# JeffWang987/MVSTER

Measured on AMD Instinct MI355X. Metric: depth-maps/sec (DTU 512×640, 5-view, 4-stage) at 1/2/4/8 MI355X, higher is better.
Workload: dtype f32; 1 GPU; DTU mid 512x640, 5 views, 4-stage cascade 8/8/4/4 hyp, B=1 eval, 1 depth map(s) per step per GPU; launch=hipGraph replay, parallelism=replicas x1, depth_maps_in_flight_per_gpu=2

## Files before the change

mvster_amd/csrc/conv_pers.hip:

```cpp
#include "conv_args.hpp"

namespace mvconv {
namespace {


#ifdef MVSTER_TIMELINE
__device__ unsigned long long* g_ptl = nullptr;
#define MV_PTL(k)                                                                                                       \
    do {                                                                                                                \
        __builtin_amdgcn_sched_barrier(0);                                                                              \
        if (g_ptl && lane == 0 && it < 16)                                                                              \
            g_ptl[(((size_t)(blockIdx.y * gridDim.x + blockIdx.x) * 4 + wave) * 16 + it) * 8 + (k)] =                    \
                (k) < 5 ? __builtin_amdgcn_s_memtime() : (k) == 5 ? __builtin_amdgcn_s_getreg(63492)                    \
                                                         : (k) == 6 ? __builtin_amdgcn_s_getreg(63508) : tile;          \
        __builtin_amdgcn_sched_barrier(0);                                                                              \
    } while (0)
#define MV_PPTL(k, v)                                                                                                   \
    do {                                                                                                                \
        __builtin_amdgcn_sched_barrier(0);                                                                              \
        if (g_ptl && lane == 0 && hp < 16)                                                                              \
            g_ptl[(((size_t)(blockIdx.y * gridDim.x + blockIdx.x) * 8 + wave8) * 16 + hp) * 4 + (k)] = (v);           \
        __builtin_amdgcn_sched_barrier(0);                                                                              \
    } while (0)
#else
// ... 571 lines not shown
                    const int tap = dy * kw + dx;
#pragma unroll
                    for (int c = 0; c < NCH; ++c) {
                        const f32x4v w = wl[(wbase + tap * NCH + c) * 64 + lane];
                        f32x4v A[MT];
#pragma unroll
                        for (int mt = 0; mt < MT; ++mt) A[mt] = patch[abase[mt] + c * 2 * PLANE + cbase + dy * RS + dx * 2];
#pragma unroll
                        for (int j = 0; j < 4; ++j)
#pragma unroll
                            for (int mt = 0; mt < MT; ++mt) acc[mt] = __builtin_amdgcn_mfma_f32_16x16x4f32(w[j], A[mt][j], acc[mt], 0, 0, 0);
                    }
                }
            wbase += kh * kw * NCH;
#pragma unroll
            for (int mt = 0; mt < MT; ++mt) {
                f32x4v v = acc[mt];
#pragma unroll
                for (int j = 0; j < 4; ++j) {
                    v[j] = fmaf(v[j], scv[j], shv[j]);
                    if (a.relu) v[j] = fmaxf(v[j], 0.0f);
                    if (SKIP) v[j] += skv[mt][j];
                }
                __builtin_amdgcn_raw_buffer_store_b128(__builtin_bit_cast(u32x4v, v), out_rsrc, ooff[mt], 0, MV_STORE_AUX);
            }
        }
        __builtin_amdgcn_s_waitcnt(0xc07f);
        __builtin_amdgcn_s_barrier();
    }
}

#ifdef MVSTER_PROBES
template <int MT, int NT, int KW, int SW, int NCH, int KD, bool WREG, int PF, bool SKIP>
__global__ void __launch_bounds__(512) conv_pp_kernel(ConvArgs a, PersArgs p) {
    using G = PersGeom<MT, KW, SW, KD>;
    constexpr int TY = G::TY, KH = G::KH, PW = G::PW, PH = G::PH, PWH = G::PWH, PLANE = G::PLANE, NBLK = G::NBLK;
    constexpr int NTAP = KD * KH * KW, TAPS2D = KH * KW;
    constexpr int BUF = NCH * 2 * PLANE;
    constexpr int NI = NCH * 2 * NBLK;
    constexpr int NIW = (NI + 3) / 4;
    constexpr int CIN = NCH * 16;
    extern __shared__ __attribute__((aligned(16))) float lds_raw[];
    const int lane = threadIdx.x & 63;
    const int wave8 = __builtin_amdgcn_readfirstlane(threadIdx.x >> 6);
    const int grp = wave8 >> 2;
    const int wave = wave8 & 3;
    f32x4v* const lds = reinterpret_cast<f32x4v*>(lds_raw) + grp * 2 * BUF;
    f32x4v* const scratch = reinterpret_cast<f32x4v*>(lds_raw) + 4 * BUF;
    f32x4v* const wl = scratch + 64;
    const int lm = lane & 15, lq = lane >> 4;
    const int nt0 = blockIdx.y * NT;
    const __amdgpu_buffer_rsrc_t in_rsrc =
        __builtin_amdgcn_make_buffer_rsrc(const_cast<float*>(a.in), (short)0, (int)a.in_bytes, 0x00020000);

    unsigned dbase[NIW];
    int dpos[NIW];
#pragma unroll
    for (int n = 0; n < NIW; ++n) {
        const int i = wave + 4 * n;
        const int c = i / (2 * NBLK), r = i - c * 2 * NBLK, pl = r / NBLK, blk = r - pl * NBLK;
        const int s = blk * 64 + lane;
        const int q1 = s & 1;
        int prow, px;
        if (SW == 1) {
            const int pix = s >> 1;
            prow = pix / PW;
            px = pix - prow * PW;
        } else {
            int t = s >> 1;
            const int xh = t % PWH;
            t /= PWH;
            prow = t >> 1;
            px = 2 * xh + (t & 1);
        }
        const bool valid = i < NI && prow < G::ROWS && px < PW;
        const int pz = KD == 1 ? 0 : prow / PH, py = prow - pz * PH;
        dpos[n] = px | (py << 8) | (pz << 16);
        dbase[n] = valid ? (unsigned)(((pz * a.Hi + py) * a.Wi + px) * (CIN * 4) + (c * 16 + pl * 8 + q1 * 4) * 4) : 0x80000000u;
    }

    auto decode_tile = [&](unsigned tile) -> TilePos {
        TilePos t;
        auto div = [&](unsigned n, int k) -> unsigned { return ((__umulhi(n, p.mul[k]) >> p.shr[k]) & ~p.one[k]) | (n & p.one[k]); };
        unsigned q = div(tile, 0);
        t.tx0 = (int)(tile - q * p.tiles_x) * 32;
        unsigned q2 = div(q, 1);
        t.ty0 = (int)(q - q2 * p.tiles_y) * TY;
        const unsigned q3 = div(q2, 2);
        t.zo = (int)(q2 - q3 * (unsigned)a.Do);
        t.b = (int)q3;
        return t;
    };

    auto dma_tile = [&](const TilePos& t, int buf, bool live) {
        const int iz0 = t.zo * a.sd - a.pd[0], iy0 = t.ty0 * SW - a.ph[0], ix0 = t.tx0 * SW - a.pw[0];
        const unsigned origin = (unsigned)((((t.b * a.Di + iz0) * a.Hi + iy0) * a.Wi + ix0) * (CIN * 4));
        const unsigned wi = live ? (unsigned)a.Wi : 0u;
        f32x4v* const dst0 = lds + buf * BUF;
#pragma unroll
        for (int n = 0; n < NIW; ++n) {
            const int i = wave + 4 * n;
            {
                const int ix = ix0 + (dpos[n] & 255), iy = iy0 + ((dpos[n] >> 8) & 255), iz = iz0 + (dpos[n] >> 16);
                bool ok = (unsigned)iy < (unsigned)a.Hi && (unsigned)ix < wi;
                if (KD > 1) ok = ok && (unsigned)iz < (unsigned)a.Di;
                const unsigned off = ok ? dbase[n] + origin : 0x80000000u;
                f32x4v* const dst = (NI % 4 == 0 || n + 1 < NIW || i < NI) ? dst0 + (i / NBLK) * PLANE + (i % NBLK) * 64 : scratch;
                __builtin_amdgcn_raw_ptr_buffer_load_lds(in_rsrc, (lds_void*)dst, 16, off, 0, 0, 0);
            }
        }
    };

    const unsigned nwg = gridDim.x;
    const unsigned first = xcd_remap(blockIdx.x, nwg);
    const unsigned ntl = first < p.ntiles ? (p.ntiles - first + nwg - 1) / nwg : 0u;
    const int kcount = (int)((ntl + 1u - (unsigned)grp) >> 1);
    auto tile_of = [&](int k) -> unsigned { return first + (unsigned)(2 * k + grp) * nwg; };
    if (kcount > 0) dma_tile(decode_tile(tile_of(0)), 0, true);
    if (grp == 0 && kcount > 1) dma_tile(decode_tile(tile_of(1)), 1, true);
    f32x4v wreg[WREG ? NTAP * NCH * NT : 1];
    const long wstep = (long)a.ntile_total * 256;
    if (WREG) {
#pragma unroll
        for (int s = 0; s < NTAP * NCH; ++s)
#pragma unroll
            for (int nt = 0; nt < NT; ++nt)
                wreg[s * NT + nt] = *reinterpret_cast<const f32x4v*>(a.wpk + s * wstep + ((long)(nt0 + nt) * 64 + lane) * 4);
    } else {
        const __amdgpu_buffer_rsrc_t w_rsrc = __builtin_amdgcn_make_buffer_rsrc(
            const_cast<float*>(a.wpk), (short)0, (int)(NTAP * NCH * wstep * 4), 0x00020000);
        for (int i = wave8; i < NTAP * NCH * NT; i += 8) {
            const int s = i / NT, nt = i - s * NT;
            const unsigned off = (unsigned)((s * wstep + (long)(nt0 + nt) * 256) * 4) + lane * 16;
            __builtin_amdgcn_raw_ptr_buffer_load_lds(w_rsrc, (lds_void*)(wl + i * 64), 16, off, 0, 0, 0);
        }
    }
    f32x4v scv[NT], shv[NT];
#pragma unroll
    for (int nt = 0; nt < NT; ++nt) {
        const int n0 = (nt0 + nt) * 16 + lq * 4;
        scv[nt] = *reinterpret_cast<const f32x4v*>(a.scale + n0);
        shv[nt] = *reinterpret_cast<const f32x4v*>(a.shift + n0);
    }
    int abase[MT];
#pragma unroll
    for (int mt = 0; mt < MT; ++mt) {
        const int t = wave * MT + mt;
        const int row = t >> 1, x = (t & 1) * 16 + lm;
        const int rs = G::ROWSLOTS;
        abase[mt] = (SW == 1 ? row * rs + x * 2 : row * 2 * rs + x * 2) + (lq >> 1) * PLANE + (lq & 1);
    }
    const __amdgpu_buffer_rsrc_t out_rsrc =
        __builtin_amdgcn_make_buffer_rsrc(a.out, (short)0, (int)p.out_bytes, 0x00020000);
    const __amdgpu_buffer_rsrc_t skip_rsrc = __builtin_amdgcn_make_buffer_rsrc(
        const_cast<float*>(SKIP ? a.skip : a.in), (short)0, SKIP ? (int)p.out_bytes : 0, 0x00020000);
    unsigned obase[MT];
    int orc[MT];
#pragma unroll
    for (int mt = 0; mt < MT; ++mt) {
        const int t = wave * MT + mt;
        const int row = t >> 1, col = (t & 1) * 16 + lm;
        orc[mt] = row | (col << 8);
        obase[mt] = (unsigned)((row * a.Wo + col) * a.cout + nt0 * 16 + lq * 4) * 4u;
    }
    auto tap_off = [&](int kz, int ky, int kx) -> int {
        const int prow = kz * PH + ky;
        return SW == 1 ? prow * G::ROWSLOTS + kx * 2 : prow * G::ROWSLOTS + (kx & 1) * PWH * 2 + (kx >> 1) * 2;
    };

    __syncthreads();

    f32x4v pacc[MT][NT], pskv[MT][NT];
    unsigned pooff[MT];
#pragma unroll
    for (int mt = 0; mt < MT; ++mt) {
        pooff[mt] = 0x80000000u;
#pragma unroll
        for (int nt = 0; nt < NT; ++nt) pacc[mt][nt] = pskv[mt][nt] = (f32x4v){0.f, 0.f, 0.f, 0.f};
    }
    auto epilogue = [&](const f32x4v (&accv)[MT][NT], const f32x4v (&skvv)[MT][NT], const unsigned (&off)[MT]) {
#pragma unroll
        for (int mt = 0; mt < MT; ++mt) {
#pragma unroll
            for (int nt = 0; nt < NT; ++nt) {
                f32x4v v = accv[mt][nt];
#pragma unroll
                for (int j = 0; j < 4; ++j) {
                    v[j] = fmaf(v[j], scv[nt][j], shv[nt][j]);
                    if (a.relu) v[j] = fmaxf(v[j], 0.0f);
                    if (SKIP) v[j] += skvv[mt][nt][j];
                }
                __builtin_amdgcn_raw_buffer_store_b128(__builtin_bit_cast(u32x4v, v), out_rsrc, off[mt] + nt * 64, 0, MV_STORE_AUX);
            }
        }
    };

    f32x4v skvN[MT][NT];
    unsigned ooffN[MT];
    TilePos here = decode_tile(kcount > 0 ? tile_of(0) : 0u);
#pragma unroll
    for (int mt = 0; mt < MT; ++mt) ooffN[mt] = 0x80000000u;
    const int nhalf = 2 * (int)((ntl + 1u) >> 1) + 1;
    {
        const unsigned oorigin = (unsigned)((((here.b * a.Do + here.zo) * a.Ho + here.ty0) * a.Wo + here.tx0) * a.cout) * 4u;
#pragma unroll
        for (int mt = 0; mt < MT; ++mt) {
            const bool ok = grp == 0 && kcount > 0 && here.ty0 + (orc[mt] & 255) < a.Ho && here.tx0 + (orc[mt] >> 8) < a.Wo;
            ooffN[mt] = ok ? obase[mt] + oorigin : 0x80000000u;
#pragma unroll
            for (int nt = 0; nt < NT; ++nt)
                skvN[mt][nt] = SKIP ? __builtin_bit_cast(f32x4v, __builtin_amdgcn_raw_buffer_load_b128(skip_rsrc, ooffN[mt] + nt * 64, 0, 0))
                                    : (f32x4v){0.f, 0.f, 0.f, 0.f};
        }
    }
    for (int hp = 0; hp < nhalf; ++hp) {
        MV_PPTL(0, __builtin_amdgcn_s_memtime());
        MV_PPTL(3, __builtin_amdgcn_s_getreg(63492));
        if ((hp & 1) == grp) {
            const int k = (hp - grp) >> 1;
            if (k < kcount) {
                const int cur = k & 1;
                f32x4v acc[MT][NT];
#pragma unroll
                for (int mt = 0; mt < MT; ++mt)
#pragma unroll
                    for (int nt = 0; nt < NT; ++nt) acc[mt][nt] = (f32x4v){0.f, 0.f, 0.f, 0.f};
                const f32x4v* patch = lds + cur * BUF;
                const int kz_lo = KD == 1 ? 0 : max(0, a.pd[0] - here.zo * a.sd), kz_hi = KD == 1 ? 1 : min(KD, a.Di + a.pd[0] - here.zo * a.sd);
#pragma unroll
                for (int kz = 0; kz < KD; ++kz) {
                    if (kz < kz_lo || kz >= kz_hi) continue;
                    f32x4v A[PF + 1][NCH][MT], Bv[PF + 1][NCH][NT];
                    auto load_tap = [&](int t2, f32x4v (&Aa)[NCH][MT], f32x4v (&Bb)[NCH][NT]) {
                        const int ky = t2 / KW, kx = t2 - ky * KW;
                        const int to = tap_off(kz, ky, kx);
                        const int tap = kz * TAPS2D + t2;
#pragma unroll
                        for (int c = 0; c < NCH; ++c) {
#pragma unroll
                            for (int mt = 0; mt < MT; ++mt) Aa[c][mt] = patch[abase[mt] + c * 2 * PLANE + to];
#pragma unroll
                            for (int nt = 0; nt < NT; ++nt)
                                Bb[c][nt] = WREG ? wreg[(tap * NCH + c) * NT + nt] : wl[((tap * NCH + c) * NT + nt) * 64 + lane];
                        }
                    };
#pragma unroll
                    for (int t2 = 0; t2 < PF && t2 < TAPS2D; ++t2) load_tap(t2, A[t2 % (PF + 1)], Bv[t2 % (PF + 1)]);
#pragma unroll
                    for (int t2 = 0; t2 < TAPS2D; ++t2) {
                        if (t2 + PF < TAPS2D) load_tap(t2 + PF, A[(t2 + PF) % (PF + 1)], Bv[(t2 + PF) % (PF + 1)]);
#pragma unroll
                        for (int c = 0; c < NCH; ++c)
#pragma unroll
                            for (int j = 0; j < 4; ++j)
#pragma unroll
                                for (int mt = 0; mt < MT; ++mt)
#pragma unroll
                                    for (int nt = 0; nt < NT; ++nt)
                                        acc[mt][nt] = __builtin_amdgcn_mfma_f32_16x16x4f32(Bv[t2 % (PF + 1)][c][nt][j], A[t2 % (PF + 1)][c][mt][j],
                                                                                           acc[mt][nt], 0, 0, 0);
                    }
                }
#pragma unroll
                for (int mt = 0; mt < MT; ++mt) {
                    pooff[mt] = ooffN[mt];
#pragma unroll
                    for (int nt = 0; nt < NT; ++nt) {
                        pacc[mt][nt] = acc[mt][nt];
                        pskv[mt][nt] = skvN[mt][nt];
                    }
                }
            }
            __builtin_amdgcn_s_waitcnt(0xc07f);
            MV_PPTL(2, k < kcount ? 1 : 0);
        } else {
            const int kn = (hp + 1 - grp) >> 1;
            epilogue(pacc, pskv, pooff);
#pragma unroll
            for (int mt = 0; mt < MT; ++mt) pooff[mt] = 0x80000000u;
            __builtin_amdgcn_sched_barrier(0);
            const bool have = kn < kcount;
            here = decode_tile(have ? tile_of(kn) : 0u);
            const unsigned oorigin = (unsigned)((((here.b * a.Do + here.zo) * a.Ho + here.ty0) * a.Wo + here.tx0) * a.cout) * 4u;
#pragma unroll
            for (int mt = 0; mt < MT; ++mt) {
                const bool ok = have && here.ty0 + (orc[mt] & 255) < a.Ho && here.tx0 + (orc[mt] >> 8) < a.Wo;
                ooffN[mt] = ok ? obase[mt] + oorigin : 0x80000000u;
#pragma unroll
                for (int nt = 0; nt < NT; ++nt)
                    skvN[mt][nt] = SKIP ? __builtin_bit_cast(f32x4v, __builtin_amdgcn_raw_buffer_load_b128(skip_rsrc, ooffN[mt] + nt * 64, 0, 0))
                                        : (f32x4v){0.f, 0.f, 0.f, 0.f};
            }
            __builtin_amdgcn_sched_barrier(0);
            const bool more = kn + 1 < kcount;
            dma_tile(decode_tile(more ? tile_of(kn + 1) : 0u), (kn + 1) & 1, more);
            MV_PPTL(2, __builtin_amdgcn_s_memtime());
            asm volatile("s_waitcnt vmcnt(%0)" ::"n"(MT * NT * (SKIP ? 2 : 1) + NIW) : "memory");
        }
        MV_PPTL(1, __builtin_amdgcn_s_memtime());
        __builtin_amdgcn_s_barrier();
    }
}
#endif

template <int NCH, int MT>
__global__ void __launch_bounds__(256) conv1x1_pers_kernel(ConvArgs a, unsigned ngroups, unsigned mtot, unsigned out_bytes) {
    constexpr int CIN = NCH * 16;
    extern __shared__ __attribute__((aligned(16))) float lds_raw[];
    f32x4v* const wl = reinterpret_cast<f32x4v*>(lds_raw);
    const int ntile = a.ntile_total;
    f32x4v* const ssl = wl + NCH * ntile * 64;
    const int lane = threadIdx.x & 63;
    const int wave = __builtin_amdgcn_readfirstlane(threadIdx.x >> 6);
    const int lm = lane & 15, lq = lane >> 4;
    const __amdgpu_buffer_rsrc_t in_rsrc =
        __builtin_amdgcn_make_buffer_rsrc(const_cast<float*>(a.in), (short)0, (int)a.in_bytes, 0x00020000);
    const __amdgpu_buffer_rsrc_t out_rsrc = __builtin_amdgcn_make_buffer_rsrc(a.out, (short)0, (int)out_bytes, 0x00020000);
    const __amdgpu_buffer_rsrc_t skip_rsrc = __builtin_amdgcn_make_buffer_rsrc(
        const_cast<float*>(a.skip_mode ? a.skip : a.in), (short)0,
        a.skip_mode == 1 ? (int)out_bytes : a.skip_mode == 2 ? (int)(out_bytes / 4) : 0, 0x00020000);
    {
        const __amdgpu_buffer_rsrc_t w_rsrc =
            __builtin_amdgcn_make_buffer_rsrc(const_cast<float*>(a.wpk), (short)0, NCH * ntile * 1024, 0x00020000);
        for (int i = wave; i < NCH * ntile; i += 4) {
            const unsigned off = (unsigned)(i * 1024 + lane * 16);
            f32x4v* const dst = wl + i * 64;
            __builtin_amdgcn_raw_ptr_buffer_load_lds(w_rsrc, (lds_void*)dst, 16, off, 0, 0, 0);
        }
        for (int i = threadIdx.x; i < ntile * 4; i += 256) {
            ssl[i] = *reinterpret_cast<const f32x4v*>(a.scale + i * 4);
            ssl[ntile * 4 + i] = *reinterpret_cast<const f32x4v*>(a.shift + i * 4);
        }
    }
    auto load_group = [&](unsigned g, f32x4v (&A)[MT][NCH], unsigned (&vox)[MT]) {
#pragma unroll
        for (int mt = 0; mt < MT; ++mt) {
            const unsigned m = ((g * 4 + wave) * MT + mt) * 16 + lm;
            vox[mt] = m;
#pragma unroll
            for (int c = 0; c < NCH; ++c) {
                const unsigned off = m < mtot ? (m * CIN + c * 16 + lq * 4) * 4u : 0x80000000u;
                A[mt][c] = __builtin_bit_cast(f32x4v, __builtin_amdgcn_raw_buffer_load_b128(in_rsrc, off, 0, 0));
            }
        }
    };
    f32x4v A[MT][NCH], An[MT][NCH];
    unsigned vox[MT], voxn[MT];
    struct Up {
        unsigned o00, o01, o10, o11;
        mv::Lerp ly, lx;
    } up[MT];
    unsigned g = blockIdx.x;
    if (g < ngroups) load_group(g, A, vox);
    __syncthreads();
    const unsigned cout4 = (unsigned)a.cout * 4u;
    for (; g < ngroups; g += gridDim.x) {
        const unsigned gn = g + gridDim.x < ngroups ? g + gridDim.x : g;
        load_group(gn, An, voxn);
        if (a.skip_mode == 2) {
            const int hh = a.HoF / 2, wh = a.WoF / 2;
#pragma unroll
            for (int mt = 0; mt < MT; ++mt) {
                const unsigned m = vox[mt] < mtot ? vox[mt] : 0u;
                const unsigned t = fast_div(m, (unsigned)a.Wo, a.div_mul[0], a.div_shr[0]);
                const int ox = (int)(m - t * (unsigned)a.Wo);
                const unsigned b = fast_div(t, (unsigned)a.Ho, a.div_mul[1], a.div_shr[1]);
                const int oy = (int)(t - b * (unsigned)a.Ho);
                up[mt].ly = mv::make_lerp(oy, hh, a.HoF);
                up[mt].lx = mv::make_lerp(ox, wh, a.WoF);
                const unsigned base = b * (unsigned)(hh * wh);
                up[mt].o00 = (base + up[mt].ly.i0 * wh + up[mt].lx.i0) * cout4;
                up[mt].o01 = (base + up[mt].ly.i0 * wh + up[mt].lx.i1) * cout4;
                up[mt].o10 = (base + up[mt].ly.i1 * wh + up[mt].lx.i0) * cout4;
                up[mt].o11 = (base + up[mt].ly.i1 * wh + up[mt].lx.i1) * cout4;
            }
        }
        f32x4v Bv[NCH];
#pragma unroll
        for (int c = 0; c < NCH; ++c) Bv[c] = wl[(c * ntile) * 64 + lane];
        for (int nt = 0; nt < ntile; ++nt) {
            f32x4v Bn[NCH];
            const int ntn = nt + 1 < ntile ? nt + 1 : nt;
#pragma unroll
            for (int c = 0; c < NCH; ++c) Bn[c] = wl[(c * ntile + ntn) * 64 + lane];
            const f32x4v sc = ssl[nt * 4 + lq], sh = ssl[ntile * 4 + nt * 4 + lq];
            f32x4v acc[MT];
#pragma unroll
            for (int mt = 0; mt < MT; ++mt) acc[mt] = (f32x4v){0.f, 0.f, 0.f, 0.f};
#pragma unroll
            for (int c = 0; c < NCH; ++c)
#pragma unroll
                for (int j = 0; j < 4; ++j)
#pragma unroll
                    for (int mt = 0; mt < MT; ++mt)
                        acc[mt] = __builtin_amdgcn_mfma_f32_16x16x4f32(Bv[c][j], A[mt][c][j], acc[mt], 0, 0, 0);
            const unsigned n0 = (unsigned)(nt * 16 + lq * 4);
#pragma unroll
            for (int mt = 0; mt < MT; ++mt) {
                const unsigned off = (n0 < (unsigned)a.cout && vox[mt] < mtot) ? vox[mt] * cout4 + n0 * 4u : 0x80000000u;
                f32x4v v = acc[mt];
#pragma unroll
                for (int j = 0; j < 4; ++j) {
                    v[j] = fmaf(v[j], sc[j], sh[j]);
                    if (a.relu) v[j] = fmaxf(v[j], 0.0f);
                }
                if (a.skip_mode == 1) {
                    const f32x4v k = __builtin_bit_cast(f32x4v, __builtin_amdgcn_raw_buffer_load_b128(skip_rsrc, off, 0, 0));
#pragma unroll
                    for (int j = 0; j < 4; ++j) v[j] += k[j];
                } else if (a.skip_mode == 2) {
                    const bool ok = n0 < (unsigned)a.cout && vox[mt] < mtot;
                    const unsigned c4 = n0 * 4u;
                    const f32x4v k00 = __builtin_bit_cast(f32x4v, __builtin_amdgcn_raw_buffer_load_b128(skip_rsrc, ok ? up[mt].o00 + c4 : 0x80000000u, 0, 0));
                    const f32x4v k01 = __builtin_bit_cast(f32x4v, __builtin_amdgcn_raw_buffer_load_b128(skip_rsrc, ok ? up[mt].o01 + c4 : 0x80000000u, 0, 0));
                    const f32x4v k10 = __builtin_bit_cast(f32x4v, __builtin_amdgcn_raw_buffer_load_b128(skip_rsrc, ok ? up[mt].o10 + c4 : 0x80000000u, 0, 0));
                    const f32x4v k11 = __builtin_bit_cast(f32x4v, __builtin_amdgcn_raw_buffer_load_b128(skip_rsrc, ok ? up[mt].o11 + c4 : 0x80000000u, 0, 0));
#pragma unroll
                    for (int j = 0; j < 4; ++j) v[j] = mv::bilerp(up[mt].ly, up[mt].lx, k00[j], k01[j], k10[j], k11[j]) + v[j];
                }
                __builtin_amdgcn_raw_buffer_store_b128(__builtin_bit_cast(u32x4v, v), out_rsrc, off, 0, MV_STORE_AUX);
            }
#pragma unroll
            for (int c = 0; c < NCH; ++c) Bv[c] = Bn[c];
        }
#pragma unroll
        for (int mt = 0; mt < MT; ++mt) {
            vox[mt] = voxn[mt];
#pragma unroll
            for (int c = 0; c < NCH; ++c) A[mt][c] = An[mt][c];
        }
    }
}


template <int MT, int NT, int KW, int SW, int NCH, int KD, bool WREG, int PF, bool SKIP, bool LD>
int launch_pers(const ConvArgs& a, int wpc, hipStream_t s) {
    using G = PersGeom<MT, KW, SW, KD>;
    constexpr int NTAP = KD * KW * KW;
    const size_t lds = (size_t)(2 * NCH * 2 * G::PLANE + 64 + (WREG ? 0 : NTAP * NCH * NT * 64)) * 16;
    if (lds > 160 * 1024) return MVSTER_ERR_UNSUPPORTED;
    auto kern = conv_pers_kernel<MT, NT, KW, SW, NCH, KD, WREG, PF, SKIP, LD>;
    static unsigned long attr_done = 0;
    if (lds > 64 * 1024 && !allow_big_lds(reinterpret_cast<const void*>(kern), attr_done)) return MVSTER_ERR_LAUNCH;
    const int g_num_cu = num_cus();
    if (g_num_cu <= 0) return MVSTER_ERR_LAUNCH;
    PersArgs p;
    if (!fill_pers_args(a, G::TY, p)) return MVSTER_ERR_UNSUPPORTED;
    const long ntiles = p.ntiles;
    p.prio = (wpc >> 4) & 1;
    wpc &= 15;
    int by_lds = (int)((160 * 1024) / lds);
    int per_cu = wpc > 0 ? wpc : (by_lds > 3 ? 3 : by_lds);
    if (per_cu > by_lds) per_cu = by_lds;
    if (per_cu < 1) per_cu = 1;
    const int ny = a.ntile_total / NT;
    long gmax = (long)g_num_cu * per_cu / ny;
    if (gmax < 1) gmax = 1;
    const long rounds = (ntiles + gmax - 1) / gmax;
    const long gx = (ntiles + rounds - 1) / rounds;
    MV_NOTE_KERNEL("conv_pers_kernel<%d, %d, %d, %d, %d, %d, %s, %d, %s, %s>", MT, NT, KW, SW, NCH, KD, WREG ? "true" : "false", PF,
                   SKIP ? "true" : "false", LD ? "true" : "false");
    hipLaunchKernelGGL(kern, dim3((unsigned)gx, ny, 1), dim3(LD ? 512 : 256), lds, s, a, p);
    return mv_check_launch();
}

template <int NCH, bool SKIP, int KS>
int launch_tpers(const ConvArgs& a, int wpc, hipStream_t s) {
    using G = PersGeom<2, KS == 5 ? 3 : 2, 1, 1>;
    const size_t lds = (size_t)(2 * NCH * 2 * G::PLANE + 64 + (KS == 5 ? 25 : 9) * NCH * 64) * 16;
    if (lds > 160 * 1024) return MVSTER_ERR_UNSUPPORTED;
    auto kern = conv_tpers_kernel<NCH, SKIP, KS>;
    static unsigned long attr_done = 0;
    if (lds > 64 * 1024 && !allow_big_lds(reinterpret_cast<const void*>(kern), attr_done)) return MVSTER_ERR_LAUNCH;
    const int ncu = num_cus();
    if (ncu <= 0) return MVSTER_ERR_LAUNCH;
    PersArgs p;
    if (!fill_pers_args(a, G::TY, p)) return MVSTER_ERR_UNSUPPORTED;
    const long ntiles = p.ntiles;
    wpc &= 15;
    const int by_lds = (int)((160 * 1024) / lds);
    int per_cu = wpc > 0 ? wpc : 2;
    if (per_cu > by_lds) per_cu = by_lds;
    if (per_cu > 2) per_cu = 2;
    long gmax = (long)ncu * per_cu / a.ntile_total;
    if (gmax < 1) gmax = 1;
    const long rounds = (ntiles + gmax - 1) / gmax;
    const long gx = (ntiles + rounds - 1) / rounds;
    MV_NOTE_KERNEL("conv_tpers_kernel<%d, %s, %d>", NCH, SKIP ? "true" : "false", KS);
    hipLaunchKernelGGL(kern, dim3((unsigned)gx, a.ntile_total, 1), dim3(512), lds, s, a, p);
    return mv_check_launch();
}

template <int KW, bool SKIP>
int launch_pers8(const ConvArgs& a, int wpc, hipStream_t s) {
    using G = PersGeom<2, KW, 2, 1>;
    const size_t lds = (size_t)(2 * G::PLANE + 64) * 16;
    auto kern = conv_pers8_kernel<KW, SKIP>;
    static unsigned long attr_done = 0;
    if (lds > 64 * 1024 && !allow_big_lds(reinterpret_cast<const void*>(kern), attr_done)) return MVSTER_ERR_LAUNCH;
    const int ncu = num_cus();
    if (ncu <= 0) return MVSTER_ERR_LAUNCH;
    PersArgs p;
    if (!fill_pers_args(a, G::TY, p)) return MVSTER_ERR_UNSUPPORTED;
    const long ntiles = p.ntiles;
    wpc &= 15;
    const int by_lds = (int)((160 * 1024) / lds);
    int per_cu = wpc > 0 ? wpc : 2;
    if (per_cu > by_lds) per_cu = by_lds;
    if (per_cu > 3) per_cu = 3;
    const long gmax = (long)ncu * per_cu;
    const long rounds = (ntiles + gmax - 1) / gmax;
    const long gx = (ntiles + rounds - 1) / rounds;
    MV_NOTE_KERNEL("conv_pers8_kernel<%d, %s>", KW, SKIP ? "true" : "false");
    hipLaunchKernelGGL(kern, dim3((unsigned)gx, 1, 1), dim3(512), lds, s, a, p);
    return mv_check_launch();
}

#ifdef MVSTER_PROBES
template <int MT, int NT, int KW, int SW, int NCH, int KD, bool WREG, int PF, bool SKIP>
int launch_pp(const ConvArgs& a, hipStream_t s) {
    using G = PersGeom<MT, KW, SW, KD>;
    constexpr int NTAP = KD * KW * KW;
    const size_t lds = (size_t)(4 * NCH * 2 * G::PLANE + 64 + (WREG ? 0 : NTAP * NCH * NT * 64)) * 16;
    if (lds > 160 * 1024) return MVSTER_ERR_UNSUPPORTED;
    auto kern = conv_pp_kernel<MT, NT, KW, SW, NCH, KD, WREG, PF, SKIP>;
    static unsigned long attr_done = 0;
    if (!allow_big_lds(reinterpret_cast<const void*>(kern), attr_done)) return MVSTER_ERR_LAUNCH;
    const int g_num_cu = num_cus();
    if (g_num_cu <= 0) return MVSTER_ERR_LAUNCH;
    PersArgs p;
    if (!fill_pers_args(a, G::TY, p)) return MVSTER_ERR_UNSUPPORTED;
    const long ntiles = p.ntiles;
    const int ny = a.ntile_total / NT;
    long gmax = (long)g_num_cu / ny;
    if (gmax < 1) gmax = 1;
    long per = (ntiles + gmax - 1) / gmax;
    if (per > 1 && (per & 1)) ++per;
    const long gx = (ntiles + per - 1) / per;
    MV_NOTE_KERNEL("conv_pp_kernel<%d, %d, %d, %d, %d, %d, %s, %d, %s>", MT, NT, KW, SW, NCH, KD, WREG ? "true" : "false", PF,
                   SKIP ? "true" : "false");
    hipLaunchKernelGGL(kern, dim3((unsigned)gx, ny, 1), dim3(512), lds, s, a, p);
    return mv_check_launch();
}
#endif

}

#ifdef MVSTER_TIMELINE
extern "C" int mvster_debug_pers_timeline(void* buf) {
    return hipMemcpyToSymbol(HIP_SYMBOL(g_ptl), &buf, sizeof(buf)) == hipSuccess ? MVSTER_OK : MVSTER_ERR_LAUNCH;
}
#endif

namespace {
template <int NCH, int MT>
int launch_1x1(const ConvArgs& a, int wpc, hipStream_t s) {
    const size_t lds = (size_t)(NCH * a.ntile_total * 64 + 2 * a.ntile_total * 4) * 16;
    const long mtot = (long)a.B * a.Do * a.Ho * a.Wo;
    const long out_bytes = mtot * a.cout * 4;
    if (lds > 160 * 1024 || a.in_bytes >= (1u << 31) || out_bytes >= (1L << 31) || a.cout % 4 != 0) return MVSTER_ERR_UNSUPPORTED;
    auto kern = conv1x1_pers_kernel<NCH, MT>;
    static unsigned long attr_done = 0;
    if (!allow_big_lds(reinterpret_cast<const void*>(kern), attr_done)) return MVSTER_ERR_LAUNCH;
    const int g_num_cu = num_cus();
    if (g_num_cu <= 0) return MVSTER_ERR_LAUNCH;
    const long ngroups = (mtot + 64 * MT - 1) / (64 * MT);
    int by_lds = (int)((160 * 1024) / lds);
    int per_cu = wpc > 0 ? wpc : 2;
    if (per_cu > by_lds) per_cu = by_lds;
    if (per_cu > 4) per_cu = 4;
    const long gmax = (long)g_num_cu * per_cu;
    const long rounds = (ngroups + gmax - 1) / gmax;
    const long gx = (ngroups + rounds - 1) / rounds;
    MV_NOTE_KERNEL("conv1x1_pers_kernel<%d, %d>", NCH, MT);
    hipLaunchKernelGGL(kern, dim3((unsigned)gx), dim3(256), lds, s, a, (unsigned)ngroups, (unsigned)mtot, (unsigned)out_bytes);
    return mv_check_launch();
}
}

int num_cus() {
    static int n = 0;
    if (n == 0) {
        int dev = 0;
        hipDeviceProp_t prop;
        if (hipGetDevice(&dev) != hipSuccess || hipGetDeviceProperties(&prop, dev) != hipSuccess) return 0;
        n = prop.multiProcessorCount;
        if (const char* e = MV_PROBE_ENV("MVSTER_CUS")) {
            const int v = atoi(e);
            if (v > 0 && v <= n) n = v;
        }
    }
    return n;
}

int dispatch_1x1(const ConvArgs& a, int mt, int wpc, hipStream_t s) {
    if (a.nclass != 1 || a.kd[0] != 1 || a.kh[0] != 1 || a.kw[0] != 1 || a.sd != 1 || a.sh != 1 || a.sw != 1 || a.osd != 1 ||
        a.osh != 1 || a.osw != 1 || a.pd[0] != 0 || a.ph[0] != 0 || a.pw[0] != 0 || a.skip_mode > 2 || a.prob_w)
        return MVSTER_ERR_UNSUPPORTED;
    if (a.skip_mode == 2 && (a.Do != 1 || (a.HoF & 1) || (a.WoF & 1))) return MVSTER_ERR_UNSUPPORTED;
    wpc &= 15;
    if (a.cin == 64 && mt == 1) return launch_1x1<4, 1>(a, wpc, s);
    if (a.cin == 64 && mt == 2) return launch_1x1<4, 2>(a, wpc, s);
    if (a.cin == 32 && mt == 1) return launch_1x1<2, 1>(a, wpc, s);
    if (a.cin == 32 && mt == 2) return launch_1x1<2, 2>(a, wpc, s);
    if (a.cin == 32 && mt == 4) return launch_1x1<2, 4>(a, wpc, s);
    if (a.cin == 16 && mt == 2) return launch_1x1<1, 2>(a, wpc, s);
    if (a.cin == 16 && mt == 4) return launch_1x1<1, 4>(a, wpc, s);
    return MVSTER_ERR_UNSUPPORTED;
}

#ifndef MVSTER_PROBES
int dispatch_pp(const ConvArgs&, int, int, hipStream_t) { return MVSTER_ERR_UNSUPPORTED; }
#else
int dispatch_pp(const ConvArgs& a, int mt, int nt, hipStream_t s) {
    if (a.nclass != 1 || a.osd != 1 || a.osh != 1 || a.osw != 1 || a.skip_mode > 1 || a.prob_w || a.cout % 16 != 0 ||
        a.sh != a.sw || a.kh[0] != a.kw[0] || a.ntile_total % nt != 0 || mt != 2 || a.cin % 16 != 0)
        return MVSTER_ERR_UNSUPPORTED;
    const int kd = a.kd[0], kw = a.kw[0], sw = a.sw, nch = a.cin / 16;
#define MV_PP(NT_, KW_, SW_, NCH_, KD_, WREG_, PF_) \
    if (nt == NT_ && kw == KW_ && sw == SW_ && nch == NCH_ && kd == KD_)                                        \
        return a.skip_mode == 1 ? launch_pp<2, NT_, KW_, SW_, NCH_, KD_, WREG_, PF_, true>(a, s)                 \
                                : launch_pp<2, NT_, KW_, SW_, NCH_, KD_, WREG_, PF_, false>(a, s);
    MV_PP(1, 3, 1, 1, 1, true, 2)
    MV_PP(2, 3, 1, 2, 1, false, 1)
    MV_PP(2, 3, 2, 1, 1, true, 1)
#undef MV_PP
    return MVSTER_ERR_UNSUPPORTED;
}
#endif

int dispatch_pers(const ConvArgs& a, int mt, int nt, int wpc, hipStream_t s) {
    if (a.nclass == 4 && a.osd == 1 && a.osh == 2 && a.osw == 2 && a.sd == 1 && a.sh == 1 && a.sw == 1 && a.skip_mode <= 1 &&
        !a.prob_w && (a.cout % 16 == 0 || a.cout == 8) && (a.cin == 16 || a.cin == 32 || a.cin == 64) && mt == 2 && nt == 1) {
        const bool k5 = a.kh[0] == 3;
        if (k5 && a.cin == 64) return MVSTER_ERR_UNSUPPORTED;
        for (int c = 0; c < 4; ++c) {
            const int py = c >> 1, px = c & 1;
            const int kh = k5 ? 3 - py : py + 1, kw = k5 ? 3 - px : px + 1, ph = k5 ? 1 - py : 0, pw = k5 ? 1 - px : 0;
            if (a.kd[c] != 1 || a.kh[c] != kh || a.kw[c] != kw || a.pd[c] || a.ph[c] != ph || a.pw[c] != pw || a.od[c] ||
                a.oh[c] != py || a.ow[c] != px || a.nsteps[c] != kh * kw * (a.cin / 16))
                return MVSTER_ERR_UNSUPPORTED;
        }
#define MV_TP(NCH_)                                                                                                   \
    return k5 ? (a.skip_mode == 1 ? launch_tpers<NCH_, true, 5>(a, wpc, s) : launch_tpers<NCH_, false, 5>(a, wpc, s)) \
              : (a.skip_mode == 1 ? launch_tpers<NCH_, true, 3>(a, wpc, s) : launch_tpers<NCH_, false, 3>(a, wpc, s));
        if (a.cin == 16) { MV_TP(1) }
        if (a.cin == 32) { MV_TP(2) }
#undef MV_TP
        return a.skip_mode == 1 ? launch_tpers<4, true, 3>(a, wpc, s) : launch_tpers<4, false, 3>(a, wpc, s);
    }
    if (a.nclass != 1 || a.osd != 1 || a.osh != 1 || a.osw != 1 || a.skip_mode > 1 || a.prob_w || a.cout % 16 != 0 ||
        a.sh != a.sw || a.kh[0] != a.kw[0] || a.ntile_total % nt != 0 || mt != 2)
        return MVSTER_ERR_UNSUPPORTED;
    const int kd = a.kd[0], kw = a.kw[0], sw = a.sw, nch = a.cin / 16;
    if (a.cin == 8 && a.cout == 16 && sw == 2 && kd == 1 && a.sd == 1 && nt == 1 && (kw == 3 || kw == 5) && a.ph[0] == kw / 2 &&
        a.pw[0] == kw / 2) {
        if (kw == 5) return a.skip_mode == 1 ? launch_pers8<5, true>(a, wpc, s) : launch_pers8<5, false>(a, wpc, s);
        return a.skip_mode == 1 ? launch_pers8<3, true>(a, wpc, s) : launch_pers8<3, false>(a, wpc, s);
    }
    if (a.cin % 16 != 0) return MVSTER_ERR_UNSUPPORTED;
#define MV_P(NT_, KW_, SW_, NCH_, KD_, WREG_, PF_) MV_Q(2, NT_, KW_, SW_, NCH_, KD_, WREG_, PF_)
    const bool ld = (wpc & 32) != 0;
#define MV_Q(MT_, NT_, KW_, SW_, NCH_, KD_, WREG_, PF_) \
    if (mt == MT_ && nt == NT_ && kw == KW_ && sw == SW_ && nch == NCH_ && kd == KD_) {                            \
        if (ld) {                                                                                                  \
              \
            if constexpr (SW_ == 2)                                                                                \
                return a.skip_mode == 1 ? launch_pers<MT_, NT_, KW_, SW_, NCH_, KD_, WREG_, PF_, true, true>(a, wpc, s)   \
                                        : launch_pers<MT_, NT_, KW_, SW_, NCH_, KD_, WREG_, PF_, false, true>(a, wpc, s); \
            return MVSTER_ERR_UNSUPPORTED;                                                                         \
        }                                                                                                          \
        return a.skip_mode == 1 ? launch_pers<MT_, NT_, KW_, SW_, NCH_, KD_, WREG_, PF_, true, false>(a, wpc, s)   \
                                : launch_pers<MT_, NT_, KW_, SW_, NCH_, KD_, WREG_, PF_, false, false>(a, wpc, s);  \
    }
    MV_P(1, 3, 1, 1, 1, true, 2)
    MV_P(2, 3, 1, 2, 1, false, 1)
    MV_P(1, 3, 1, 2, 1, false, 1)
    MV_P(1, 3, 1, 4, 1, false, 1)
    MV_P(2, 5, 2, 1, 1, false, 1)
    MV_P(1, 3, 1, 1, 3, false, 2)
    MV_P(2, 3, 2, 1, 1, false, 1)
#undef MV_P
#undef MV_Q
    return MVSTER_ERR_UNSUPPORTED;
}

}
```

Measured before the change: 1148 depth-maps/s.

## Prefetch skip tensors one tile ahead and specialize 1x1 conv per skip mode

Restructures the persistent 1x1 conv kernel so the skip/residual loads (plain add or 4-tap bilinear upsample) for the next output-channel tile are issued before the current tile's MFMAs. Weights are double-buffered in ping-pong registers and the skip mode becomes a compile-time template parameter, which removes per-tile branches. The prefetch of the next group's activations also moves after the first tile's loads. The launcher now caps blocks per CU by the occupancy the register count allows, since the extra in-flight registers may lower occupancy.

Measured after the change: 1151 depth-maps/s, median of 4. Within noise of the previous version (+0.2%).

```diff
diff --git a/mvster_amd/csrc/conv_pers.hip b/mvster_amd/csrc/conv_pers.hip
--- a/mvster_amd/csrc/conv_pers.hip
+++ b/mvster_amd/csrc/conv_pers.hip
@@ -897,6 +897,11 @@
     }
 }
 #endif
+
+template <int V>
+struct SkipTag {
+    static constexpr int value = V;
+};
 
 template <int NCH, int MT>
 __global__ void __launch_bounds__(256) conv1x1_pers_kernel(ConvArgs a, unsigned ngroups, unsigned mtot, unsigned out_bytes) {
@@ -949,9 +954,87 @@
     if (g < ngroups) load_group(g, A, vox);
     __syncthreads();
     const unsigned cout4 = (unsigned)a.cout * 4u;
+    auto load_skip = [&](auto mode, int nt, auto& K) {
+        constexpr int SM = decltype(mode)::value;
+        const unsigned n0 = (unsigned)(nt * 16 + lq * 4);
+#pragma unroll
+        for (int mt = 0; mt < MT; ++mt) {
+            const bool ok = n0 < (unsigned)a.cout && vox[mt] < mtot;
+            const unsigned c4 = n0 * 4u;
+            if constexpr (SM == 1) {
+                K[mt][0] = __builtin_bit_cast(f32x4v, __builtin_amdgcn_raw_buffer_load_b128(skip_rsrc, ok ? vox[mt] * cout4 + c4 : 0x80000000u, 0, 0));
+            } else if constexpr (SM == 2) {
+                K[mt][0] = __builtin_bit_cast(f32x4v, __builtin_amdgcn_raw_buffer_load_b128(skip_rsrc, ok ? up[mt].o00 + c4 : 0x80000000u, 0, 0));
+                K[mt][1] = __builtin_bit_cast(f32x4v, __builtin_amdgcn_raw_buffer_load_b128(skip_rsrc, ok ? up[mt].o01 + c4 : 0x80000000u, 0, 0));
+                K[mt][2] = __builtin_bit_cast(f32x4v, __builtin_amdgcn_raw_buffer_load_b128(skip_rsrc, ok ? up[mt].o10 + c4 : 0x80000000u, 0, 0));
+                K[mt][3] = __builtin_bit_cast(f32x4v, __builtin_amdgcn_raw_buffer_load_b128(skip_rsrc, ok ? up[mt].o11 + c4 : 0x80000000u, 0, 0));
+            }
+        }
+    };
+    auto tile = [&](auto mode, auto pf, int nt, const f32x4v (&Bc)[NCH], f32x4v (&Bx)[NCH], const auto& Kc, auto& Kx) {
+        constexpr int SM = decltype(mode)::value;
+        const int ntile = a.ntile_total;
+        if constexpr (decltype(pf)::value != 0) {
+#pragma unroll
+            for (int c = 0; c < NCH; ++c) Bx[c] = wl[(c * ntile + nt + 1) * 64 + lane];
+            load_skip(mode, nt + 1, Kx);
+        }
+        __builtin_amdgcn_sched_barrier(0);
+        const f32x4v sc = ssl[nt * 4 + lq], sh = ssl[ntile * 4 + nt * 4 + lq];
+        f32x4v acc[MT];
+#pragma unroll
+        for (int mt = 0; mt < MT; ++mt) acc[mt] = (f32x4v){0.f, 0.f, 0.f, 0.f};
+#pragma unroll
+        for (int c = 0; c < NCH; ++c)
+#pragma unroll
+            for (int j = 0; j < 4; ++j)
+#pragma unroll
+                for (int mt = 0; mt < MT; ++mt)
+                    acc[mt] = __builtin_amdgcn_mfma_f32_16x16x4f32(Bc[c][j], A[mt][c][j], acc[mt], 0, 0, 0);
+        if constexpr (SM != 0) __builtin_amdgcn_sched_barrier(0);
+        const unsigned n0 = (unsigned)(nt * 16 + lq * 4);
+#pragma unroll
+        for (int mt = 0; mt < MT; ++mt) {
+            const unsigned off = (n0 < (unsigned)a.cout && vox[mt] < mtot) ? vox[mt] * cout4 + n0 * 4u : 0x80000000u;
+            f32x4v v = acc[mt];
+#pragma unroll
+            for (int j = 0; j < 4; ++j) {
+                v[j] = fmaf(v[j], sc[j], sh[j]);
+                if (a.relu) v[j] = fmaxf(v[j], 0.0f);
+            }
+            if constexpr (SM == 1) {
+#pragma unroll
+                for (int j = 0; j < 4; ++j) v[j] += Kc[mt][0][j];
+            } else if constexpr (SM == 2) {
+#pragma unroll
+                for (int j = 0; j < 4; ++j)
+                    v[j] = mv::bilerp(up[mt].ly, up[mt].lx, Kc[mt][0][j], Kc[mt][1][j], Kc[mt][2][j], Kc[mt][3][j]) + v[j];
+            }
+            __builtin_amdgcn_raw_buffer_store_b128(__builtin_bit_cast(u32x4v, v), out_rsrc, off, 0, MV_STORE_AUX);
+        }
+    };
+    auto run_group = [&](auto mode, unsigned gn) {
+        constexpr int NK = decltype(mode)::value == 2 ? 4 : 1;
+        const int ntile = a.ntile_total;
+        f32x4v B0[NCH], B1[NCH], K0[MT][NK], K1[MT][NK];
+#pragma unroll
+        for (int c = 0; c < NCH; ++c) B0[c] = wl[(c * ntile) * 64 + lane];
+        load_skip(mode, 0, K0);
+        load_group(gn, An, voxn);
+        int nt = 0;
+        for (; nt + 2 < ntile; nt += 2) {
+            tile(mode, SkipTag<1>{}, nt, B0, B1, K0, K1);
+            tile(mode, SkipTag<1>{}, nt + 1, B1, B0, K1, K0);
+        }
+        if (nt + 2 == ntile) {
+            tile(mode, SkipTag<1>{}, nt, B0, B1, K0, K1);
+            tile(mode, SkipTag<0>{}, nt + 1, B1, B0, K1, K0);
+        } else {
+            tile(mode, SkipTag<0>{}, nt, B0, B1, K0, K1);
+        }
+    };
     for (; g < ngroups; g += gridDim.x) {
         const unsigned gn = g + gridDim.x < ngroups ? g + gridDim.x : g;
-        load_group(gn, An, voxn);
         if (a.skip_mode == 2) {
             const int hh = a.HoF / 2, wh = a.WoF / 2;
 #pragma unroll
@@ -970,54 +1053,9 @@
                 up[mt].o11 = (base + up[mt].ly.i1 * wh + up[mt].lx.i1) * cout4;
             }
         }
-        f32x4v Bv[NCH];
-#pragma unroll
-        for (int c = 0; c < NCH; ++c) Bv[c] = wl[(c * ntile) * 64 + lane];
-        for (int nt = 0; nt < ntile; ++nt) {
-            f32x4v Bn[NCH];
-            const int ntn = nt + 1 < ntile ? nt + 1 : nt;
-#pragma unroll
-            for (int c = 0; c < NCH; ++c) Bn[c] = wl[(c * ntile + ntn) * 64 + lane];
-            const f32x4v sc = ssl[nt * 4 + lq], sh = ssl[ntile * 4 + nt * 4 + lq];
-            f32x4v acc[MT];
-#pragma unroll
-            for (int mt = 0; mt < MT; ++mt) acc[mt] = (f32x4v){0.f, 0.f, 0.f, 0.f};
-#pragma unroll
-            for (int c = 0; c < NCH; ++c)
-#pragma unroll
-                for (int j = 0; j < 4; ++j)
-#pragma unroll
-                    for (int mt = 0; mt < MT; ++mt)
-                        acc[mt] = __builtin_amdgcn_mfma_f32_16x16x4f32(Bv[c][j], A[mt][c][j], acc[mt], 0, 0, 0);
-            const unsigned n0 = (unsigned)(nt * 16 + lq * 4);
-#pragma unroll
-            for (int mt = 0; mt < MT; ++mt) {
-                const unsigned off = (n0 < (unsigned)a.cout && vox[mt] < mtot) ? vox[mt] * cout4 + n0 * 4u : 0x80000000u;
-                f32x4v v = acc[mt];
-#pragma unroll
-                for (int j = 0; j < 4; ++j) {
-                    v[j] = fmaf(v[j], sc[j], sh[j]);
-                    if (a.relu) v[j] = fmaxf(v[j], 0.0f);
-                }
-                if (a.skip_mode == 1) {
-                    const f32x4v k = __builtin_bit_cast(f32x4v, __builtin_amdgcn_raw_buffer_load_b128(skip_rsrc, off, 0, 0));
-#pragma unroll
-                    for (int j = 0; j < 4; ++j) v[j] += k[j];
-                } else if (a.skip_mode == 2) {
-                    const bool ok = n0 < (unsigned)a.cout && vox[mt] < mtot;
-                    const unsigned c4 = n0 * 4u;
-                    const f32x4v k00 = __builtin_bit_cast(f32x4v, __builtin_amdgcn_raw_buffer_load_b128(skip_rsrc, ok ? up[mt].o00 + c4 : 0x80000000u, 0, 0));
-                    const f32x4v k01 = __builtin_bit_cast(f32x4v, __builtin_amdgcn_raw_buffer_load_b128(skip_rsrc, ok ? up[mt].o01 + c4 : 0x80000000u, 0, 0));
-                    const f32x4v k10 = __builtin_bit_cast(f32x4v, __builtin_amdgcn_raw_buffer_load_b128(skip_rsrc, ok ? up[mt].o10 + c4 : 0x80000000u, 0, 0));
-                    const f32x4v k11 = __builtin_bit_cast(f32x4v, __builtin_amdgcn_raw_buffer_load_b128(skip_rsrc, ok ? up[mt].o11 + c4 : 0x80000000u, 0, 0));
-#pragma unroll
-                    for (int j = 0; j < 4; ++j) v[j] = mv::bilerp(up[mt].ly, up[mt].lx, k00[j], k01[j], k10[j], k11[j]) + v[j];
-                }
-                __builtin_amdgcn_raw_buffer_store_b128(__builtin_bit_cast(u32x4v, v), out_rsrc, off, 0, MV_STORE_AUX);
-            }
-#pragma unroll
-            for (int c = 0; c < NCH; ++c) Bv[c] = Bn[c];
-        }
+        if (a.skip_mode == 2) run_group(SkipTag<2>{}, gn);
+        else if (a.skip_mode == 1) run_group(SkipTag<1>{}, gn);
+        else run_group(SkipTag<0>{}, gn);
 #pragma unroll
         for (int mt = 0; mt < MT; ++mt) {
             vox[mt] = voxn[mt];
@@ -1160,9 +1198,12 @@
     const int g_num_cu = num_cus();
     if (g_num_cu <= 0) return MVSTER_ERR_LAUNCH;
     const long ngroups = (mtot + 64 * MT - 1) / (64 * MT);
+    static int by_regs = 0;
+    if (by_regs == 0 && (hipOccupancyMaxActiveBlocksPerMultiprocessor(&by_regs, kern, 256, 0) != hipSuccess || by_regs < 1)) by_regs = 1;
     int by_lds = (int)((160 * 1024) / lds);
     int per_cu = wpc > 0 ? wpc : 2;
     if (per_cu > by_lds) per_cu = by_lds;
+    if (per_cu > by_regs) per_cu = by_regs;
     if (per_cu > 4) per_cu = 4;
     const long gmax = (long)g_num_cu * per_cu;
     const long rounds = (ngroups + gmax - 1) / gmax;
```
